# AIRI-Institute/HairFastGAN

Measured on AMD Instinct MI355X. Metric: stylegan2_generator_fwd_1024_images_per_sec, higher is better.
Workload: dtype f32 tensors + f32 accumulate; conv products as 3 fp16 MFMAs on (hi,lo)-split operands (fp32-class); 1 GPU; StyleGAN2 1024^2 generator forward (range 0->8), random W+, fresh noise per layer, HIP modulated-conv + upfirdn2d kernels (BASELINE.json configs[1]); batch_per_gpu=8, global_batch=8, parallelism=replica x1, weights=synthetic closed-form (oracle/synth.py), conv_precision=f16x3

## Files before the change

hairfastgan_amd/csrc/hf_common.h:

```cpp
#pragma once
#include <hip/hip_runtime.h>

#include "../../include/hairfast_hip.h"

#define HF_WAVE 64

#ifndef HF_DYN_LDS
#define HF_DYN_LDS extern __shared__ __attribute__((aligned(16))) unsigned char hf_dyn_lds[]
#endif

#ifndef HF_OPAQUE_F32
#define HF_OPAQUE_F32(v) asm volatile("" : "+v"(v))
#define HF_OPAQUE_I32(v) asm volatile("" : "+v"(v))
#endif

#ifndef HF_BARRIER_KEEP_DEFINED
#define HF_BARRIER_KEEP_DEFINED
__device__ __forceinline__ void hf_glds16_raw(const float *gsrc_lane, float *lds_wave_base) {
  const unsigned base = __builtin_amdgcn_readfirstlane(
      (unsigned)(__UINTPTR_TYPE__)(__attribute__((address_space(3))) void *)lds_wave_base);
  asm volatile("s_mov_b32 m0, %0\n\ts_nop 0\n\tglobal_load_lds_dwordx4 %1, off" ::"s"(base), "v"(gsrc_lane) : "memory");
}
__device__ __forceinline__ unsigned hf_lds_addr(const void *lds_ptr) {
  return (unsigned)(__UINTPTR_TYPE__)(__attribute__((address_space(3))) const void *)lds_ptr;
}
__device__ __forceinline__ void hf_glds16_raw_s(const void *gsrc_uniform, unsigned lane_byte_offset,
                                                unsigned lds_wave_addr) {
  const unsigned base = __builtin_amdgcn_readfirstlane(lds_wave_addr);
  const unsigned long long g = (unsigned long long)gsrc_uniform;
  const unsigned g_hi = (unsigned)__builtin_amdgcn_readfirstlane((int)(g >> 32));
  const unsigned g_lo = (unsigned)__builtin_amdgcn_readfirstlane((int)(unsigned)g);
  const unsigned long long gs = ((unsigned long long)g_hi << 32) | g_lo;
  asm volatile("s_mov_b32 m0, %0\n\ts_nop 0\n\tglobal_load_lds_dwordx4 %1, %2" ::"s"(base), "v"(lane_byte_offset), "s"(gs)
               : "memory");
}
__device__ __forceinline__ void hf_glds16_raw_s_if(bool active, const void *gsrc_uniform, unsigned lane_byte_offset,
                                                   unsigned lds_wave_addr) {
  if (active) hf_glds16_raw_s(gsrc_uniform, lane_byte_offset, lds_wave_addr);
}
__device__ __forceinline__ void hf_barrier_lds() { asm volatile("s_waitcnt lgkmcnt(0)\n\ts_barrier" ::: "memory"); }
template <int NYOUNG>
__device__ __forceinline__ void hf_barrier_keep_young() {
  static_assert(NYOUNG >= 0 && NYOUNG < 64, "vmcnt is a 6-bit counter");
  asm volatile("s_waitcnt vmcnt(%0) lgkmcnt(0)\n\ts_barrier" ::"n"(NYOUNG) : "memory");
}
#endif

#ifndef HF_GLDS16_DEFINED
#define HF_GLDS16_DEFINED
__device__ __forceinline__ void hf_glds16(const float *gsrc_lane, float *lds_wave_base) {
  __builtin_amdgcn_global_load_lds((const __attribute__((address_space(1))) void *)gsrc_lane,
                                   (__attribute__((address_space(3))) void *)lds_wave_base, 16, 0, 0);
}
__device__ __forceinline__ void hf_glds4(const float *gsrc_lane, float *lds_wave_base) {
  __builtin_amdgcn_global_load_lds((const __attribute__((address_space(1))) void *)gsrc_lane,
                                   (__attribute__((address_space(3))) void *)lds_wave_base, 4, 0, 0);
}
__device__ __forceinline__ void hf_glds16_if(bool active, const float *gsrc_lane, float *lds_wave_base) {
  if (active) hf_glds16(gsrc_lane, lds_wave_base);
}
__device__ __forceinline__ void hf_glds4_if(bool active, const float *gsrc_lane, float *lds_wave_base) {
  if (active) hf_glds4(gsrc_lane, lds_wave_base);
}
#endif

#ifdef HF_WANT_F16_SPLIT
#define HF_F16_MAX 65504.0f
static __device__ unsigned int hf_f16_overflow_dev;
static inline unsigned int hf_f16_overflow_read_tu(int reset) {
  unsigned int v = 0, z = 0;
  if (hipMemcpyFromSymbol(&v, HIP_SYMBOL(hf_f16_overflow_dev), sizeof(v)) != hipSuccess) return 0xffffffffu;
  if (reset) (void)hipMemcpyToSymbol(HIP_SYMBOL(hf_f16_overflow_dev), &z, sizeof(z));
  return v;
}
__device__ __forceinline__ void hf_split_f16(float v, _Float16 &hi, _Float16 &lo, bool &ovf) {
  HF_OPAQUE_F32(v);
  ovf = ovf || !(fabsf(v) <= 2.0f * HF_F16_MAX);
  const float vh = fminf(fmaxf(v, -HF_F16_MAX), HF_F16_MAX);
  hi = (_Float16)vh;
  const float r = v - (float)hi;
  lo = (_Float16)fminf(fmaxf(r, -HF_F16_MAX), HF_F16_MAX);
}
__device__ __forceinline__ void hf_note_overflow(bool ovf) {
  if (ovf) atomicAdd(&hf_f16_overflow_dev, 1u);
}
typedef _Float16 hf_half4 __attribute__((ext_vector_type(4)));
#ifndef HF_WAVE_ANY_DEFINED
#define HF_WAVE_ANY_DEFINED
__device__ __forceinline__ bool hf_wave_any(bool p) { return __any((int)p) != 0; }
#endif
__device__ __forceinline__ void hf_split4_f16(const float (&vin)[4], hf_half4 &h, hf_half4 &l, bool &ovf) {
  float v[4];
#pragma unroll
  for (int k = 0; k < 4; ++k) {
    v[k] = vin[k];
    HF_OPAQUE_F32(v[k]);
  }
  const float m = fmaxf(fmaxf(fabsf(v[0]), fabsf(v[1])), fmaxf(fabsf(v[2]), fabsf(v[3])));
  if (hf_wave_any(!(m <= HF_F16_MAX))) {
#pragma unroll
    for (int k = 0; k < 4; ++k) {
      _Float16 hv, lv;
      hf_split_f16(v[k], hv, lv, ovf);
      h[k] = hv;
      l[k] = lv;
    }
  } else {
    typedef _Float16 hf_half2_ __attribute__((ext_vector_type(2)));
    typedef float hf_float2_ __attribute__((ext_vector_type(2)));
#pragma unroll
    for (int p = 0; p < 2; ++p) {
      hf_float2_ x;
      x.x = v[2 * p];
      x.y = v[2 * p + 1];
      const hf_half2_ hh = __builtin_convertvector(x, hf_half2_);
      const hf_float2_ r = x - __builtin_convertvector(hh, hf_float2_);
      const hf_half2_ ll = __builtin_convertvector(r, hf_half2_);
      h[2 * p] = hh.x;
      h[2 * p + 1] = hh.y;
      l[2 * p] = ll.x;
      l[2 * p + 1] = ll.y;
    }
  }
}
#endif

#ifndef HF_LANE_SHIFT_DEFINED
#define HF_LANE_SHIFT_DEFINED
__device__ __forceinline__ float hf_lane_up(float v) {
  return __builtin_bit_cast(float, __builtin_amdgcn_update_dpp(0, __builtin_bit_cast(int, v), 0x138, 0xf, 0xf, true));
}
__device__ __forceinline__ float hf_lane_down(float v) {
  return __builtin_bit_cast(float, __builtin_amdgcn_update_dpp(0, __builtin_bit_cast(int, v), 0x130, 0xf, 0xf, true));
}
#endif

#ifndef HF_HALF_SWAP_DEFINED
#define HF_HALF_SWAP_DEFINED
__device__ __forceinline__ void hf_half_swap(unsigned &a, unsigned &b) {
  const auto r = __builtin_amdgcn_permlane32_swap(a, b, false, false);
  a = r[0];
  b = r[1];
}
#endif

static inline int hf_launch_status() {
  return hipGetLastError() == hipSuccess ? HF_OK : HF_E_LAUNCH;
}

static inline int hf_cdiv(long long a, long long b) { return (int)((a + b - 1) / b); }

__device__ __forceinline__ float hf_lrelu(float v, float alpha, float scale) {
  return (v > 0.0f ? v : v * alpha) * scale;
}

__device__ __forceinline__ float hf_wave_sum(float v) {
#pragma unroll
  for (int m = 32; m >= 1; m >>= 1) v += __shfl_xor(v, m, HF_WAVE);
  return v;
}
```

hairfastgan_amd/csrc/upfirdn2d.hip:

```cpp
#define HF_WANT_F16_SPLIT
#include "hf_common.h"

#pragma clang fp contract(on)

namespace {

constexpr int kMaxTaps = 8;

__global__ __launch_bounds__(256) void upfirdn2d_generic(
    float *__restrict__ out, const float *__restrict__ in, const float *__restrict__ kernel, int in_h,
    int in_w, int out_h, int out_w, int kh, int kw, int up_x, int up_y, int down_x, int down_y, int pad_x0,
    int pad_y0, long long total) {
  HF_DYN_LDS;
  float *kf = reinterpret_cast<float *>(hf_dyn_lds);
  for (int i = threadIdx.x; i < kh * kw; i += blockDim.x) {
    int ky = i / kw, kx = i - ky * kw;
    kf[i] = kernel[(kh - 1 - ky) * kw + (kw - 1 - kx)];
  }
  __syncthreads();
  long long stride = (long long)gridDim.x * blockDim.x;
  for (long long idx = (long long)blockIdx.x * blockDim.x + threadIdx.x; idx < total; idx += stride) {
    int ox = (int)(idx % out_w);
    long long t = idx / out_w;
    int oy = (int)(t % out_h);
    long long plane = t / out_h;
    const float *src = in + plane * (long long)in_h * in_w;
    float acc = 0.0f;
    for (int ky = 0; ky < kh; ++ky) {
      int uy = oy * down_y + ky - pad_y0;
      if (uy < 0 || uy % up_y) continue;
      int iy = uy / up_y;
      if (iy >= in_h) continue;
      for (int kx = 0; kx < kw; ++kx) {
        int ux = ox * down_x + kx - pad_x0;
        if (ux < 0 || ux % up_x) continue;
        int ix = ux / up_x;
        if (ix >= in_w) continue;
        acc = fmaf(src[(long long)iy * in_w + ix], kf[ky * kw + kx], acc);
      }
    }
    out[idx] = acc;
  }
}

constexpr int kBlurCols = 64;
constexpr int kBlurSegs = 4;
constexpr int kRowsPerThread = 32;

__global__ __launch_bounds__(256) void blur4x4_noise_bias_act(
    float *__restrict__ out, const float *__restrict__ in, const float *__restrict__ kernel4x4,
    const float *__restrict__ noise, const float *__restrict__ noise_w, long long noise_bstride,
    const float *__restrict__ bias, int channels, int in_h, int in_w, int in_pitch, float alpha, float scale) {
  const int out_h = in_h - 1, out_w = in_w - 1;
  const int ox = blockIdx.x * kBlurCols + threadIdx.x;
  const int oy0 = (blockIdx.y * kBlurSegs + threadIdx.y) * kRowsPerThread;
  const int plane = blockIdx.z;
  if (ox >= out_w || oy0 >= out_h) return;

  float kf[4][4];
#pragma unroll
  for (int ky = 0; ky < 4; ++ky)
#pragma unroll
    for (int kx = 0; kx < 4; ++kx) kf[ky][kx] = kernel4x4[(3 - ky) * 4 + (3 - kx)];

  const float *src = in + (long long)plane * in_h * in_pitch;
  float *dst = out + (long long)plane * out_h * out_w;
  const int c = plane % channels;
  const int b = plane / channels;
  const float bc = bias ? bias[c] : 0.0f;
  const float nw = noise ? noise_w[0] : 0.0f;
  const float *nz = noise ? noise + (long long)b * noise_bstride : nullptr;

  bool cv[4];
#pragma unroll
  for (int j = 0; j < 4; ++j) cv[j] = (ox - 1 + j) >= 0 && (ox - 1 + j) < in_w;

  float win[7][4];
  auto load_row = [&](int iy, float (&row)[4]) {
    const bool rv = iy >= 0 && iy < in_h;
    const float *p = src + (long long)iy * in_pitch + (ox - 1);
#pragma unroll
    for (int j = 0; j < 4; ++j) row[j] = (rv && cv[j]) ? p[j] : 0.0f;
  };
#pragma unroll
  for (int r = 0; r < 3; ++r) load_row(oy0 - 1 + r, win[r]);

  const int oy_end = min(oy0 + kRowsPerThread, out_h);
  for (int oy = oy0; oy < oy_end; oy += 4) {
#pragma unroll
    for (int r = 0; r < 4; ++r) load_row(oy + 2 + r, win[3 + r]);
#pragma unroll
    for (int q = 0; q < 4; ++q) {
      if (oy + q < oy_end) {
        float acc = 0.0f;
#pragma unroll
        for (int r = 0; r < 4; ++r)
#pragma unroll
          for (int j = 0; j < 4; ++j) acc = fmaf(win[q + r][j], kf[r][j], acc);
        if (nz) acc = fmaf(nw, nz[(long long)(oy + q) * out_w + ox], acc);
        if (bias) acc = hf_lrelu(acc + bc, alpha, scale);
        dst[(long long)(oy + q) * out_w + ox] = acc;
      }
    }
#pragma unroll
    for (int r = 0; r < 3; ++r)
#pragma unroll
      for (int j = 0; j < 4; ++j) win[r][j] = win[r + 4][j];
  }
}


struct __attribute__((packed, aligned(4))) f32x4u {
  float x, y, z, w;
};

__global__ __launch_bounds__(256) void blur4x4_noise_bias_act_vec4(
    float *__restrict__ out, const float *__restrict__ in, const float *__restrict__ kernel4x4,
    const float *__restrict__ noise, const float *__restrict__ noise_w, long long noise_bstride,
    const float *__restrict__ bias, int channels, int in_h, int in_w, int in_pitch, float alpha, float scale,
    int rows_per_thread) {
  const int out_h = in_h - 1, out_w = in_w - 1;
  const int c0 = (blockIdx.x * blockDim.x + threadIdx.x) * 4;
  const int oy0 = (blockIdx.y * blockDim.y + threadIdx.y) * rows_per_thread;
  const int plane = blockIdx.z;
  const bool active = c0 < out_w && oy0 < out_h;
  const int lane = (threadIdx.y * blockDim.x + threadIdx.x) & 63;
  const bool nb_left = lane > 0 && threadIdx.x > 0;
  const bool nb_right = lane < 63 && threadIdx.x + 1 < blockDim.x && c0 + 4 < out_w;

  float kf[4][4];
#pragma unroll
  for (int ky = 0; ky < 4; ++ky)
#pragma unroll
    for (int kx = 0; kx < 4; ++kx) kf[ky][kx] = kernel4x4[(3 - ky) * 4 + (3 - kx)];

  const float *src = in + (long long)plane * in_h * in_pitch;
  float *dst = out + (long long)plane * out_h * out_w;
  const int c = plane % channels;
  const int b = plane / channels;
  const float bc = bias ? bias[c] : 0.0f;
  const float nw = noise ? noise_w[0] : 0.0f;
  const float *nz = noise ? noise + (long long)b * noise_bstride : nullptr;

  float win[6][7];
  struct RowRaw {
    f32x4u m;
    float e0, e5, e6;
  };
  auto issue = [&](int iy) {
    RowRaw r;
    const bool rv = active && iy >= 0 && iy < in_h;
    const float *p = src + (long long)iy * in_pitch + c0;
    r.m = f32x4u{0.f, 0.f, 0.f, 0.f};
    if (rv) r.m = *reinterpret_cast<const f32x4u *>(p);
    r.e0 = (!nb_left && rv && c0 > 0) ? p[-1] : 0.0f;
    r.e5 = (!nb_right && rv && c0 + 4 < in_w) ? p[4] : 0.0f;
    r.e6 = (!nb_right && rv && c0 + 5 < in_w) ? p[5] : 0.0f;
    return r;
  };
  auto finish = [&](const RowRaw &r, float (&row)[7]) {
    row[1] = r.m.x; row[2] = r.m.y; row[3] = r.m.z; row[4] = r.m.w;
    const float l = __shfl_up(r.m.w, 1, 64), r0 = __shfl_down(r.m.x, 1, 64), r1 = __shfl_down(r.m.y, 1, 64);
    row[0] = nb_left ? l : r.e0;
    row[5] = nb_right ? r0 : r.e5;
    row[6] = nb_right ? r1 : r.e6;
  };
  {
    RowRaw a = issue(oy0 - 1), b2 = issue(oy0), c2 = issue(oy0 + 1), d2 = issue(oy0 + 2);
    finish(a, win[0]); finish(b2, win[1]); finish(c2, win[2]); finish(d2, win[3]);
  }

  const int oy_end = min(oy0 + rows_per_thread, out_h);
  RowRaw nx0 = issue(oy0 + 3), nx1 = issue(oy0 + 4);
  for (int oy = oy0; oy < oy0 + rows_per_thread; oy += 2) {
    finish(nx0, win[4]);
    finish(nx1, win[5]);
    nx0 = issue(oy + 5);
    nx1 = issue(oy + 6);
#pragma unroll
    for (int q2 = 0; q2 < 2; ++q2) {
      float acc[4] = {0.f, 0.f, 0.f, 0.f};
#pragma unroll
      for (int r = 0; r < 4; ++r)
#pragma unroll
        for (int j = 0; j < 4; ++j)
#pragma unroll
          for (int q = 0; q < 4; ++q) acc[q] = fmaf(win[q2 + r][q + j], kf[r][j], acc[q]);
      const int oyy = oy + q2;
      if (active && oyy < oy_end) {
        if (nz) {
          const float4 z = *reinterpret_cast<const float4 *>(nz + (long long)oyy * out_w + c0);
          acc[0] = fmaf(nw, z.x, acc[0]); acc[1] = fmaf(nw, z.y, acc[1]);
          acc[2] = fmaf(nw, z.z, acc[2]); acc[3] = fmaf(nw, z.w, acc[3]);
        }
        if (bias) {
#pragma unroll
          for (int q = 0; q < 4; ++q) acc[q] = hf_lrelu(acc[q] + bc, alpha, scale);
        }
        *reinterpret_cast<float4 *>(dst + (long long)oyy * out_w + c0) =
            make_float4(acc[0], acc[1], acc[2], acc[3]);
      }
    }
#pragma unroll
    for (int r = 0; r < 4; ++r)
#pragma unroll
      for (int j = 0; j < 7; ++j) win[r][j] = win[r + 2][j];
  }
}

}

extern "C" int hf_upfirdn2d_f32(float *out, const float *in, const float *kernel, int major, int in_h,
                                int in_w, int kh, int kw, int up_x, int up_y, int down_x, int down_y,
                                int pad_x0, int pad_x1, int pad_y0, int pad_y1, void *stream) {
  if (!out || !in || !kernel || major <= 0 || in_h <= 0 || in_w <= 0 || kh <= 0 || kw <= 0 ||
      kh > kMaxTaps || kw > kMaxTaps || up_x <= 0 || up_y <= 0 || down_x <= 0 || down_y <= 0)
    return HF_E_INVALID;
  const int full_h = in_h * up_y + pad_y0 + pad_y1 - kh;
  const int full_w = in_w * up_x + pad_x0 + pad_x1 - kw;
  if (full_h < 0 || full_w < 0) return HF_E_INVALID;
  const int out_h = full_h / down_y + 1, out_w = full_w / down_x + 1;
  const long long total = (long long)major * out_h * out_w;
  long long g = (total + 255) / 256;
  if (g > 4096) g = 4096;
  hipLaunchKernelGGL(upfirdn2d_generic, dim3((int)g), dim3(256), kMaxTaps * kMaxTaps * sizeof(float),
                     (hipStream_t)stream, out, in, kernel, in_h, in_w, out_h, out_w, kh, kw, up_x, up_y,
                     down_x, down_y, pad_x0, pad_y0, total);
  return hf_launch_status();
}

typedef _Float16 hf_half8 __attribute__((ext_vector_type(8)));

__global__ __launch_bounds__(512) void blur4x4_split8(hf_half8 *__restrict__ hi, hf_half8 *__restrict__ lo,
                                                      const float *__restrict__ in,
                                                      const float *__restrict__ kernel4x4,
                                                      const float *__restrict__ noise,
                                                      const float *__restrict__ noise_w, long long noise_bstride,
                                                      const float *__restrict__ bias,
                                                      const float *__restrict__ s_next, int channels, int in_h,
                                                      int in_w, int in_pitch, float alpha, float scale,
                                                      int rows_per_thread) {
  const int out_h = in_h - 1, out_w = in_w - 1;
  const int lane = threadIdx.x & 63;
  const int wv = blockIdx.x * (blockDim.x >> 6) + (threadIdx.x >> 6);
  const int ix = 61 * wv + lane - 1;
  const int ox = ix + 1;
  const int oy0 = blockIdx.y * rows_per_thread;
  const int cblocks = channels >> 3;
  const int b = blockIdx.z / cblocks, cb = blockIdx.z - b * cblocks;
  if (61 * wv >= out_w || oy0 >= out_h) return;
  const bool produces = lane < 61 && ox < out_w;

  float kf[4][4];
#pragma unroll
  for (int ky = 0; ky < 4; ++ky)
#pragma unroll
    for (int kx = 0; kx < 4; ++kx) kf[ky][kx] = kernel4x4[(3 - ky) * 4 + (3 - kx)];
  float bc[8], sv[8];
#pragma unroll
  for (int k = 0; k < 8; ++k) {
    bc[k] = bias ? bias[cb * 8 + k] : 0.0f;
    sv[k] = s_next ? s_next[(long long)b * channels + cb * 8 + k] : 1.0f;
  }
  const float nw = noise ? noise_w[0] : 0.0f;
  const float *nz = noise ? noise + (long long)b * noise_bstride : nullptr;
  const long long iplane = (long long)in_h * in_pitch;
  const bool colv = ix >= 0 && ix < in_w;
  const float *src = in + ((long long)b * channels + cb * 8) * iplane + (colv ? ix : 0);
  const int oxc = min(ox, out_w - 1);
  hf_half8 *hp = hi + ((long long)b * cblocks + cb) * out_h * out_w + oxc;
  hf_half8 *lp = lo + ((long long)b * cblocks + cb) * out_h * out_w + oxc;

  const int oy_end = min(oy0 + rows_per_thread, out_h);
  float acc[8][4];
#pragma unroll
  for (int k = 0; k < 8; ++k)
#pragma unroll
    for (int t = 0; t < 4; ++t) acc[k][t] = 0.0f;

  const int n_end = (oy_end - oy0) + 3;
  for (int n0 = 0; n0 < n_end; n0 += 4) {
    float own[4][8];
#pragma unroll
    for (int u = 0; u < 4; ++u) {
      const int iy = oy0 - 1 + n0 + u;
      const bool rv = colv && iy >= 0 && iy < in_h && (n0 + u) < n_end;
      const long long ro = (long long)min(max(iy, 0), in_h - 1) * in_pitch;
#pragma unroll
      for (int k = 0; k < 8; ++k) {
        const float v = src[k * iplane + ro];
        own[u][k] = rv ? v : 0.0f;
      }
    }
#pragma unroll
    for (int u = 0; u < 4; ++u) {
      const int n = n0 + u;
      if (n < n_end) {
#pragma unroll
        for (int k = 0; k < 8; ++k) {
          float win[4];
          win[0] = own[u][k];
          win[1] = hf_lane_down(win[0]);
          win[2] = hf_lane_down(win[1]);
          win[3] = hf_lane_down(win[2]);
#pragma unroll
          for (int r = 0; r < 4; ++r) {
            const int slot = (u - r) & 3;
            if (n - r >= 0) {
              float a = (r == 0) ? 0.0f : acc[k][slot];
#pragma unroll
              for (int j = 0; j < 4; ++j) a = fmaf(win[j], kf[r][j], a);
              acc[k][slot] = a;
            }
          }
        }
        const int oy = oy0 + n - 3;
        if (n >= 3 && oy < oy_end && produces) {
          const int slot = (u - 3) & 3;
          const float nzr = nz ? nz[(long long)oy * out_w + ox] : 0.0f;
          hf_half8 h8, l8;
          bool ovf = false;
#pragma unroll
          for (int k = 0; k < 8; ++k) {
            float v = acc[k][slot];
            if (nz) v = fmaf(nw, nzr, v);
            if (bias) v = hf_lrelu(v + bc[k], alpha, scale);
            v *= sv[k];
            _Float16 hv, lv;
            hf_split_f16(v, hv, lv, ovf);
            h8[k] = hv;
            l8[k] = lv;
          }
          hf_note_overflow(ovf);
          hp[(long long)oy * out_w] = h8;
          if (lo) lp[(long long)oy * out_w] = l8;
        }
      }
    }
  }
}

extern "C" unsigned long long hf_f16_overflow_count_blur(int reset) { return hf_f16_overflow_read_tu(reset); }

extern "C" int hf_blur_noise_bias_act_f32(float *out, const float *in, const float *kernel4x4,
                                          const float *noise, const float *noise_w,
                                          long long noise_bstride, const float *bias, int batch,
                                          int channels, int in_h, int in_w, int in_pitch, float alpha,
                                          float scale, void *stream) {
  if (!out || !in || !kernel4x4 || batch <= 0 || channels <= 0 || in_h < 2 || in_w < 2 || in_pitch < in_w ||
      (noise && !noise_w))
    return HF_E_INVALID;
  const long long planes = (long long)batch * channels;
  if (planes > 65535LL * 32768) return HF_E_INVALID;
  const int out_h = in_h - 1, out_w = in_w - 1;
  const bool aligned = ((((size_t)out) | ((size_t)noise)) & 15) == 0 && (noise_bstride & 3) == 0;
  if ((out_w & 3) == 0 && aligned) {
    int cq = 64;
    while (cq > 1 && cq * 4 >= 2 * out_w) cq >>= 1;
    const int segs = 256 / cq;
    int rpt = 32;
    while (rpt > 2 && segs * rpt >= 2 * out_h) rpt >>= 1;
    dim3 grid(hf_cdiv(out_w, cq * 4), hf_cdiv(out_h, segs * rpt), (unsigned)planes);
    hipLaunchKernelGGL(blur4x4_noise_bias_act_vec4, grid, dim3(cq, segs), 0, (hipStream_t)stream, out, in,
                       kernel4x4, noise, noise_w, noise_bstride, bias, channels, in_h, in_w, in_pitch, alpha, scale, rpt);
    return hf_launch_status();
  }
  dim3 grid(hf_cdiv(out_w, kBlurCols), hf_cdiv(out_h, kBlurSegs * kRowsPerThread), (unsigned)planes);
  hipLaunchKernelGGL(blur4x4_noise_bias_act, grid, dim3(kBlurCols, kBlurSegs), 0, (hipStream_t)stream, out,
                     in, kernel4x4, noise, noise_w, noise_bstride, bias, channels, in_h, in_w, in_pitch, alpha, scale);
  return hf_launch_status();
}

extern "C" int hf_blur_noise_bias_act_split_f16(void *out_hi, void *out_lo, const float *in, const float *kernel4x4,
                                                const float *noise, const float *noise_w, long long noise_bstride,
                                                const float *bias, const float *s_next, int batch, int channels,
                                                int in_h, int in_w, int in_pitch, float alpha, float scale,
                                                void *stream) {
  if (!out_hi || !in || !kernel4x4 || batch <= 0 || channels <= 0 || (channels & 7) || in_h < 2 || in_w < 2 ||
      in_pitch < in_w || (noise && !noise_w))
    return HF_E_INVALID;
  const long long zs = (long long)batch * (channels >> 3);
  if (zs > 65535) return HF_E_INVALID;
  const int out_h = in_h - 1, out_w = in_w - 1;
  const int waves = hf_cdiv(out_w, 61);
  int wpb = 1, waste = 1 << 30;
  for (int k = 8; k >= 1; --k) {
    const int ws = hf_cdiv(waves, k) * k - waves;
    if (ws < waste) { waste = ws; wpb = k; }
  }
  const int tx = 64 * wpb;
  int rpt = 64;
  while (rpt > 8 && (long long)hf_cdiv(waves, wpb) * hf_cdiv(out_h, rpt) * zs * wpb < 8192) rpt >>= 1;
  dim3 grid(hf_cdiv(waves, wpb), hf_cdiv(out_h, rpt), (unsigned)zs);
  hipLaunchKernelGGL(blur4x4_split8, grid, dim3(tx), 0, (hipStream_t)stream, static_cast<hf_half8 *>(out_hi),
                     static_cast<hf_half8 *>(out_lo), in, kernel4x4, noise, noise_w, noise_bstride, bias, s_next, channels,
                     in_h, in_w, in_pitch, alpha, scale, rpt);
  return hf_launch_status();
}
```

Measured before the change: 1773 images/s.

## Add two-half-wave blur kernel splitting channel groups across 32-lane halves

Adds a new blur4x4 split-f16 kernel where each 64-lane wave covers 32 output columns, with the two half-waves handling four channels each. It uses DPP lane shifts plus a small extra load for the halo, and permlane32 swaps to pack hi/lo halves into 16-byte stores. A rolling 4-row register pipeline prefetches rows two ahead. The kernel is enabled by default unless a tune bit is set, and it adds a helper that loads through a uniform scalar base with a per-lane 32-bit offset. The aim is better memory coalescing and a lower instruction count than the old kernel, which spread 61 columns per wave. The cost is redundant halo loads and possibly lower occupancy from 64-thread blocks.

```diff
diff --git a/hairfastgan_amd/csrc/hf_common.h b/hairfastgan_amd/csrc/hf_common.h
--- a/hairfastgan_amd/csrc/hf_common.h
+++ b/hairfastgan_amd/csrc/hf_common.h
@@ -135,6 +135,21 @@
 }
 #endif
 
+#ifndef HF_LOAD_UBASE_DEFINED
+#define HF_LOAD_UBASE_DEFINED
+#ifdef __HIP__
+__device__ __forceinline__ float hf_load_f32_ubase(const float *uniform_base, unsigned lane_byte_offset) {
+  unsigned long long g = (unsigned long long)uniform_base;
+  asm("" : "+s"(g));
+  return *(const __attribute__((address_space(1))) float *)(g + lane_byte_offset);
+}
+#else
+inline float hf_load_f32_ubase(const float *uniform_base, unsigned lane_byte_offset) {
+  return *reinterpret_cast<const float *>(reinterpret_cast<const char *>(uniform_base) + lane_byte_offset);
+}
+#endif
+#endif
+
 #ifndef HF_HALF_SWAP_DEFINED
 #define HF_HALF_SWAP_DEFINED
 __device__ __forceinline__ void hf_half_swap(unsigned &a, unsigned &b) {
diff --git a/hairfastgan_amd/csrc/upfirdn2d.hip b/hairfastgan_amd/csrc/upfirdn2d.hip
--- a/hairfastgan_amd/csrc/upfirdn2d.hip
+++ b/hairfastgan_amd/csrc/upfirdn2d.hip
@@ -1,5 +1,5 @@
 #define HF_WANT_F16_SPLIT
-#include "hf_common.h"
+#include "conv_common.h"
 
 #pragma clang fp contract(on)
 
@@ -340,6 +340,140 @@
   }
 }
 
+struct BlurRow4 {
+  float a[4], e[4];
+};
+typedef unsigned hf_u32x4 __attribute__((ext_vector_type(4)));
+typedef unsigned hf_u32x2 __attribute__((ext_vector_type(2)));
+
+__global__ __launch_bounds__(64) void blur4x4_split8_w32x2(hf_half8 *__restrict__ hi, hf_half8 *__restrict__ lo,
+                                                           const float *__restrict__ in,
+                                                           const float *__restrict__ kernel4x4,
+                                                           const float *__restrict__ noise,
+                                                           const float *__restrict__ noise_w, long long noise_bstride,
+                                                           const float *__restrict__ bias,
+                                                           const float *__restrict__ s_next, int channels, int in_h,
+                                                           int in_w, int in_pitch, float alpha, float scale,
+                                                           int rows_per_strip) {
+  const int out_h = in_h - 1, out_w = in_w - 1;
+  const int lane = threadIdx.x, hl = lane & 31, half = lane >> 5;
+  const int ox = 32 * blockIdx.x + hl;
+  const int ix = ox - 1;
+  const int oy0 = blockIdx.y * rows_per_strip;
+  const int cblocks = channels >> 3;
+  const int b = blockIdx.z / cblocks, cb = blockIdx.z - b * cblocks;
+  const bool produces = ox < out_w;
+
+  float kf[4][4];
+#pragma unroll
+  for (int ky = 0; ky < 4; ++ky)
+#pragma unroll
+    for (int kx = 0; kx < 4; ++kx) kf[ky][kx] = kernel4x4[(3 - ky) * 4 + (3 - kx)];
+  float bc[4], sv[4];
+#pragma unroll
+  for (int k = 0; k < 4; ++k) {
+    bc[k] = bias ? bias[cb * 8 + half * 4 + k] : 0.0f;
+    sv[k] = s_next ? s_next[(long long)b * channels + cb * 8 + half * 4 + k] : 1.0f;
+  }
+  const float nw = noise ? noise_w[0] : 0.0f;
+  const float *nz = noise ? noise + (long long)b * noise_bstride : nullptr;
+  const long long iplane = (long long)in_h * in_pitch;
+  const bool colv = ix >= 0 && ix < in_w;
+  const bool extv = hl >= 29 && ix + 3 < in_w;
+  const float *plane0 = in + ((long long)b * channels + cb * 8) * iplane;
+  const unsigned hoff = 16u * (unsigned)half * (unsigned)iplane;
+  const unsigned coff = hoff + 4u * (colv ? ix : 0), ecoff = extv ? hoff + 4u * (ix + 3) : coff;
+  const long long unit0 = ((long long)b * cblocks + cb) * out_h * out_w + min(ox, out_w - 1);
+  hf_u32x4 *dst = reinterpret_cast<hf_u32x4 *>(half ? lo : hi) + unit0;
+  const bool stores = produces && (half == 0 || lo != nullptr);
+
+  const int oy_end = min(oy0 + rows_per_strip, out_h);
+  const int n_end = (oy_end - oy0) + 3;
+  float acc[4][4];
+#pragma unroll
+  for (int k = 0; k < 4; ++k)
+#pragma unroll
+    for (int t = 0; t < 4; ++t) acc[k][t] = 0.0f;
+
+  auto issue = [&](int n, BlurRow4 &r) {
+    const float *rowp = plane0 + (long long)min(max(oy0 - 1 + n, 0), in_h - 1) * in_pitch;
+#pragma unroll
+    for (int k = 0; k < 4; ++k) {
+      r.a[k] = hf_load_f32_ubase(rowp + k * iplane, coff);
+      r.e[k] = hf_load_f32_ubase(rowp + k * iplane, ecoff);
+    }
+  };
+
+  auto consume = [&](const BlurRow4 &r, int n, int u, int nr) {
+    const int iy = oy0 - 1 + n;
+    const bool rv = iy >= 0 && iy < in_h;
+#pragma unroll
+    for (int k = 0; k < 4; ++k) {
+      float win[4];
+      const float e = (rv && extv) ? r.e[k] : 0.0f;
+      const float e1 = hf_lane_up(e), e2 = hf_lane_up(e1);
+      win[0] = (rv && colv) ? r.a[k] : 0.0f;
+      win[1] = hf_lane_down(win[0]);
+      win[2] = hf_lane_down(win[1]);
+      win[3] = hf_lane_down(win[2]);
+      win[1] = hl == 31 ? e2 : win[1];
+      win[2] = hl >= 30 ? e1 : win[2];
+      win[3] = hl >= 29 ? e : win[3];
+#pragma unroll
+      for (int rr = 0; rr < 4; ++rr) {
+        if (rr < nr) {
+          const int slot = (u - rr) & 3;
+          float a = (rr == 0) ? 0.0f : acc[k][slot];
+#pragma unroll
+          for (int j = 0; j < 4; ++j) a = fmaf(win[j], kf[rr][j], a);
+          acc[k][slot] = a;
+        }
+      }
+    }
+    const int oy = oy0 + n - 3;
+    if (nr == 4 && oy < oy_end) {
+      const int slot = (u - 3) & 3;
+      const float nzr = (nz && produces) ? nz[(long long)oy * out_w + ox] : 0.0f;
+      float v[4];
+#pragma unroll
+      for (int k = 0; k < 4; ++k) {
+        v[k] = acc[k][slot];
+        if (nz) v[k] = fmaf(nw, nzr, v[k]);
+        if (bias) v[k] = hf_lrelu(v[k] + bc[k], alpha, scale);
+        v[k] *= sv[k];
+      }
+      hf_half4 h4, l4;
+      bool ovf = false;
+      hf_split4_f16(v, h4, l4, ovf);
+      hf_note_overflow(ovf && produces);
+      const hf_u32x2 hq = __builtin_bit_cast(hf_u32x2, h4), lq = __builtin_bit_cast(hf_u32x2, l4);
+      unsigned a0 = hq.x, b0 = lq.x, a1 = hq.y, b1 = lq.y;
+      hf_half_swap(a0, b0);
+      hf_half_swap(a1, b1);
+      hf_u32x4 unit;
+      unit.x = a0; unit.y = a1; unit.z = b0; unit.w = b1;
+      if (stores) dst[(long long)oy * out_w] = unit;
+    }
+  };
+
+  BlurRow4 buf[4];
+  issue(0, buf[0]);
+  issue(1, buf[1]);
+#pragma unroll
+  for (int u = 0; u < 3; ++u) {
+    issue(u + 2, buf[(u + 2) & 3]);
+    consume(buf[u], u, u, u + 1);
+  }
+  for (int n0 = 3; n0 < n_end; n0 += 4) {
+#pragma unroll
+    for (int u = 3; u < 7; ++u) {
+      const int n = n0 + u - 3;
+      issue(n + 2, buf[(u + 2) & 3]);
+      consume(buf[u & 3], n, u & 3, 4);
+    }
+  }
+}
+
 extern "C" unsigned long long hf_f16_overflow_count_blur(int reset) { return hf_f16_overflow_read_tu(reset); }
 
 extern "C" int hf_blur_noise_bias_act_f32(float *out, const float *in, const float *kernel4x4,
@@ -382,6 +516,17 @@
   const long long zs = (long long)batch * (channels >> 3);
   if (zs > 65535) return HF_E_INVALID;
   const int out_h = in_h - 1, out_w = in_w - 1;
+  if (!(hf_detail::g_h_tune & 64) && 16LL * in_h * in_pitch + 4LL * in_pitch < (1LL << 32)) {
+    const int cw = hf_cdiv(out_w, 32);
+    if (cw > 65535) return HF_E_INVALID;
+    int rps = 32;
+    while (rps > 8 && (long long)cw * hf_cdiv(out_h, rps) * zs < 4096) rps >>= 1;
+    dim3 grid(cw, hf_cdiv(out_h, rps), (unsigned)zs);
+    hipLaunchKernelGGL(blur4x4_split8_w32x2, grid, dim3(64), 0, (hipStream_t)stream, static_cast<hf_half8 *>(out_hi),
+                       static_cast<hf_half8 *>(out_lo), in, kernel4x4, noise, noise_w, noise_bstride, bias, s_next, channels,
+                       in_h, in_w, in_pitch, alpha, scale, rps);
+    return hf_launch_status();
+  }
   const int waves = hf_cdiv(out_w, 61);
   int wpb = 1, waste = 1 << 30;
   for (int k = 8; k >= 1; --k) {
```

Result: no change. 1777 images/s, median of 6 (+0.2%).

## Add LDS-staged band kernel for split-f16 blur with noise/bias/act

Applied to the files above, without the earlier changes.

Adds a new blur kernel that stages a band of input rows for eight channels into LDS using async global-to-LDS loads, zero-pads the borders, and has four waves compute row segments from LDS with a rolling register window. It applies noise, bias, activation and scaling, and writes the hi/lo f16 split. The host dispatches to it when the pitch is aligned and the LDS fits, unless a tuning bit is set. The goal is to cut redundant global reads of overlapping rows. In exchange it uses a large dynamic LDS footprint, which lowers occupancy, and puts a sync between staging and compute.

```diff
diff --git a/hairfastgan_amd/csrc/upfirdn2d.hip b/hairfastgan_amd/csrc/upfirdn2d.hip
--- a/hairfastgan_amd/csrc/upfirdn2d.hip
+++ b/hairfastgan_amd/csrc/upfirdn2d.hip
@@ -340,7 +340,139 @@
   }
 }
 
+#ifndef HF_BLUR_BAND_ROWS
+#define HF_BLUR_BAND_ROWS 16
+#endif
+#ifndef HF_BLUR_BAND_LDS_FLOOR
+#define HF_BLUR_BAND_LDS_FLOOR 0
+#endif
+constexpr int kBandWaves = 4;
+constexpr size_t kBandLdsMax = 150 * 1024;
+
+__global__ __launch_bounds__(64 * kBandWaves, 3) void blur4x4_split8_band(
+    hf_half8 *__restrict__ hi, hf_half8 *__restrict__ lo, const float *__restrict__ in, const float *__restrict__ kernel4x4,
+    const float *__restrict__ noise, const float *__restrict__ noise_w, long long noise_bstride,
+    const float *__restrict__ bias, const float *__restrict__ s_next, int channels, int in_h, int in_w, int in_pitch,
+    float alpha, float scale, int band_rows, int sub_rows) {
+  HF_DYN_LDS;
+  float *T = reinterpret_cast<float *>(hf_dyn_lds) + 4;
+  const int out_h = in_h - 1, out_w = in_w - 1;
+  const int lane = threadIdx.x & 63, wave = threadIdx.x >> 6;
+  const int cblocks = channels >> 3;
+  const int b = blockIdx.z / cblocks, cb = blockIdx.z - b * cblocks;
+  const int oy0 = blockIdx.x * band_rows;
+  const int nrows = min(band_rows, out_h - oy0);
+  const int nr_in = nrows + 3, iy0 = oy0 - 1;
+  const int plane = nr_in * in_pitch;
+  const long long iplane = (long long)in_h * in_pitch;
+
+  {
+    const int f_lo = max(0, -iy0) * in_pitch;
+    const int f_hi = (min(in_h, iy0 + nr_in) - iy0) * in_pitch;
+    if (threadIdx.x < 4) T[(int)threadIdx.x - 4] = 0.0f;
+#pragma unroll
+    for (int cc = 0; cc < 8 / kBandWaves; ++cc) {
+      const int c = wave * (8 / kBandWaves) + cc;
+      const float *sc = in + ((long long)b * channels + cb * 8 + c) * iplane;
+      for (int k0 = 0; k0 < plane; k0 += 256) {
+        const int f = k0 + lane * 4;
+        const bool inside = f < plane;
+        const bool valid = inside && f >= f_lo && f < f_hi;
+        float *wbase = T + c * plane + k0;
+        hf_glds16_if(valid, sc + ((long long)iy0 * in_pitch + (valid ? f : f_lo)), wbase);
+        if (inside && !valid) *reinterpret_cast<float4 *>(wbase + lane * 4) = make_float4(0.f, 0.f, 0.f, 0.f);
+      }
+    }
+  }
+  __syncthreads();
+  for (int q = threadIdx.x; q < 8 * nr_in; q += 64 * kBandWaves) {
+    float *p = T + q * in_pitch + in_w;
+    for (int x = 0; x < in_pitch - in_w; ++x) p[x] = 0.0f;
+  }
+  __syncthreads();
+
+  float kf[4][4];
+#pragma unroll
+  for (int ky = 0; ky < 4; ++ky)
+#pragma unroll
+    for (int kx = 0; kx < 4; ++kx) kf[ky][kx] = kernel4x4[(3 - ky) * 4 + (3 - kx)];
+  float bc[8], sv[8];
+#pragma unroll
+  for (int k = 0; k < 8; ++k) {
+    bc[k] = bias ? bias[cb * 8 + k] : 0.0f;
+    sv[k] = s_next ? s_next[(long long)b * channels + cb * 8 + k] : 1.0f;
+  }
+  const float nw = noise ? noise_w[0] : 0.0f;
+  const float *nz = noise ? noise + (long long)b * noise_bstride : nullptr;
+
+  const int segs = (out_w + 63) >> 6;
+  int item = 0;
+  for (int ry0 = 0; ry0 < nrows; ry0 += sub_rows) {
+    for (int seg = 0; seg < segs; ++seg, ++item) {
+      if ((item & (kBandWaves - 1)) != wave) continue;
+      const int nr = min(sub_rows, nrows - ry0);
+      const int ox = seg * 64 + lane;
+      const bool produces = ox < out_w;
+      const int oxc = min(ox, out_w - 1);
+      const float *tp = T + ry0 * in_pitch + (oxc - 1);
+      const long long unit0 = (((long long)b * cblocks + cb) * out_h + oy0 + ry0) * out_w + oxc;
+      hf_half8 *hp = hi + unit0;
+      hf_half8 *lp = lo + unit0;
+      const float *nzp = nz ? nz + (long long)(oy0 + ry0) * out_w + oxc : nullptr;
+      float nzr = nzp ? nzp[0] : 0.0f;
+
+      float w[4][8][4];
+#pragma unroll
+      for (int n = 0; n < 3; ++n)
+#pragma unroll
+        for (int k = 0; k < 8; ++k)
+#pragma unroll
+          for (int j = 0; j < 4; ++j) w[n][k][j] = tp[k * plane + n * in_pitch + j];
+      for (int q0 = 0; q0 < nr; q0 += 4) {
+#pragma unroll
+        for (int u = 0; u < 4; ++u) {
+          const int q = q0 + u;
+          if (q < nr) {
+#pragma unroll
+            for (int k = 0; k < 8; ++k)
+#pragma unroll
+              for (int j = 0; j < 4; ++j) w[(u + 3) & 3][k][j] = tp[k * plane + (q + 3) * in_pitch + j];
+            const float nzc = nzr;
+            if (nzp && q + 1 < nr) nzr = nzp[(long long)(q + 1) * out_w];
+            hf_half8 h8, l8;
+            bool ovf = false;
+#pragma unroll
+            for (int k = 0; k < 8; ++k) {
+              float v = 0.0f;
+#pragma unroll
+              for (int r = 0; r < 4; ++r)
+#pragma unroll
+                for (int j = 0; j < 4; ++j) v = fmaf(w[(u + r) & 3][k][j], kf[r][j], v);
+              if (nz) v = fmaf(nw, nzc, v);
+              if (bias) v = hf_lrelu(v + bc[k], alpha, scale);
+              v *= sv[k];
+              _Float16 hv, lv;
+              hf_split_f16(v, hv, lv, ovf);
+              h8[k] = hv;
+              l8[k] = lv;
+            }
+            if (produces) {
+              hf_note_overflow(ovf);
+              hp[(long long)q * out_w] = h8;
+              if (lo) lp[(long long)q * out_w] = l8;
+            }
+          }
+        }
+      }
+    }
+  }
+}
+
 extern "C" unsigned long long hf_f16_overflow_count_blur(int reset) { return hf_f16_overflow_read_tu(reset); }
+
+namespace hf_detail {
+extern thread_local int g_h_tune;
+}
 
 extern "C" int hf_blur_noise_bias_act_f32(float *out, const float *in, const float *kernel4x4,
                                           const float *noise, const float *noise_w,
@@ -382,6 +514,21 @@
   const long long zs = (long long)batch * (channels >> 3);
   if (zs > 65535) return HF_E_INVALID;
   const int out_h = in_h - 1, out_w = in_w - 1;
+  {
+    const int band_rows = out_h < HF_BLUR_BAND_ROWS ? out_h : HF_BLUR_BAND_ROWS;
+    const size_t lds = 16 + (size_t)8 * (band_rows + 3) * in_pitch * sizeof(float);
+    const bool rows16 = (in_pitch & 3) == 0 && in_pitch > in_w && (((size_t)in) & 15) == 0;
+    if (!(hf_detail::g_h_tune & 64) && rows16 && lds <= kBandLdsMax) {
+      const int segs = hf_cdiv(out_w, 64);
+      const int sub_rows = hf_cdiv((long long)band_rows * segs, kBandWaves);
+      dim3 grid(hf_cdiv(out_h, band_rows), 1, (unsigned)zs);
+      hipLaunchKernelGGL(blur4x4_split8_band, grid, dim3(64 * kBandWaves), lds < HF_BLUR_BAND_LDS_FLOOR ? HF_BLUR_BAND_LDS_FLOOR : lds,
+                         (hipStream_t)stream, static_cast<hf_half8 *>(out_hi), static_cast<hf_half8 *>(out_lo), in, kernel4x4,
+                         noise, noise_w, noise_bstride, bias, s_next, channels, in_h, in_w, in_pitch, alpha, scale, band_rows,
+                         sub_rows);
+      return hf_launch_status();
+    }
+  }
   const int waves = hf_cdiv(out_w, 61);
   int wpb = 1, waste = 1 << 30;
   for (int k = 8; k >= 1; --k) {
```

Result: no change. 1816 images/s before, 1814 images/s after (-0.1%).
